# keeffEoghan/tendrils

Hardware: AMD Instinct MI355X
Metric: particle-steps/sec (16M particles per GPU) (higher is better)
Workload: dtype f32

## Files before the change

### include/tendrils_hip.h

```cpp
#ifndef TENDRILS_HIP_H
#define TENDRILS_HIP_H

#include <stddef.h>
#include <stdint.h>

#ifdef __cplusplus
extern "C" {
#endif

#define TH_ABI_VERSION 14

typedef int32_t th_status;
enum {
    TH_OK = 0,
    TH_ERR_INVALID = 1,
    TH_ERR_HIP = 2,
    TH_ERR_NO_DEVICE = 3,
    TH_ERR_UNSUPPORTED = 4
};

#define TH_INERT (-1000000.0f)

typedef struct th_context th_context;

// ... 224 lines not shown
    float alpha;
} th_blend_view;
th_status th_texture_upload(th_context *ctx, int32_t slot, int32_t format, const void *texels, int32_t w, int32_t h);
th_status th_texture_download(th_context *ctx, int32_t slot, void *texels);
th_status th_colormap_resize(th_context *ctx, int32_t w, int32_t h);
th_status th_colormap_shape(th_context *ctx, int32_t *w, int32_t *h);
th_status th_colormap_blend(th_context *ctx, const th_blend_view *views, int32_t n, int32_t gl_blend, int32_t clear);
th_status th_colormap_download(th_context *ctx, float *rgba);
th_status th_export_view_lines(th_context *ctx, const th_render_uniforms *u, float *lines, uint64_t capacity, uint64_t *count);
th_status th_draw_sharded(th_context *ctx, const th_deposit_uniforms *u, const th_render_uniforms *r, uint64_t *fragments);
th_status th_view_emit(th_context *ctx, const th_render_uniforms *u, uint64_t *count, void **keys_dev, void **colors_dev);
th_status th_view_merge(th_context *ctx, const void *keys_dev, const void *colors_dev, uint64_t count);
th_status th_view_device_ptr(th_context *ctx, void **dptr);
th_status th_draw_emit(th_context *ctx, const th_deposit_uniforms *u, const th_render_uniforms *r, uint64_t *count, void **keys_dev, void **colors_dev);
th_status th_draw_merge(th_context *ctx, const void *keys_dev, const void *colors_dev, uint64_t count);

typedef struct th_slot_order_info {
    int32_t sorted_buffers;
    int32_t steps_since_sort;
    uint64_t window_misses;
    uint64_t sorts;
} th_slot_order_info;
th_status th_slot_order(th_context *ctx, th_slot_order_info *out);

enum { TH_DRAW_AUTO = -1, TH_DRAW_STREAM = 0, TH_DRAW_BINS = 1 };
th_status th_draw_pipeline(th_context *ctx, int32_t which);
typedef struct th_draw_info {
    int32_t pipeline;
    int32_t reserved;
    uint64_t fragments, crowded_fragments;
    uint64_t sent_bytes, received_bytes;
} th_draw_info;
th_status th_draw_query(th_context *ctx, th_draw_info *out);

typedef struct th_flow_line_uniforms {
    float speed, rad, crestShape, speedLimit;
    float viewSize[2];
} th_flow_line_uniforms;

th_status th_flow_line_attributes(const float *points, const double *times, int32_t n, int32_t closed, int32_t capacity,
                                  int32_t *nverts, float *position, float *normal, float *miter, float *previous,
                                  float *time, float *dt);
th_status th_flow_lines(th_context *ctx, const th_flow_line_uniforms *u, const float *points, const double *times,
                        const int32_t *offsets, const int32_t *closed, int32_t nlines);

enum { TH_OPT_BUCKET = 0, TH_OPT_RESORT_STEPS = 1, TH_OPT_REBUCKET_STEPS = 2, TH_OPT_FUSE = 3, TH_OPT_GRAPH = 4,
       TH_OPT_FORCE_GENERIC = 5, TH_OPT_DRAW_REUSE = 6, TH_OPT_BINS_POOL = 7,
#ifdef TH_TESTING
       TH_OPT_INJECT_FAILURE = 8,
#endif
       TH_OPT_BINS_PAGES = 9, TH_OPT_ASYNC_SORT = 10, TH_OPT_SKIP_UNSEEN = 11, TH_OPT_SPAWN_CHUNK_ROWS = 12,
       TH_OPT_HASH_WINDOW = 13, TH_OPT_HASH_WINDOW_LAUNCHES = 14 };
th_status th_option_set(th_context *ctx, int32_t option, int64_t value);
th_status th_option_get(th_context *ctx, int32_t option, int64_t *value);

#ifdef __cplusplus
}
#endif
#endif
```

### tendrils_amd/_capi.py

```python
import ctypes as C
import os

HERE = os.path.dirname(os.path.abspath(__file__))
LIB_PATH = os.environ.get("TH_LIB") or os.path.join(HERE, "lib", "libtendrils_hip.so")

TH_OK = 0
TH_MODE_EXACT, TH_MODE_FAST = 0, 1
TH_STATE_F32, TH_STATE_F16 = 0, 1
TH_PASS_FLOW, TH_PASS_VIEW = 0, 1
TH_MAX_LINE_WIDTH = 64.0
TH_TARGET_RING, TH_TARGET_TARGETS, TH_SOURCE_FLOW, TH_SOURCE_IMAGE, TH_SOURCE_NONE = -1, -2, -3, -4, -5
TH_ERR_INVALID, TH_ERR_HIP, TH_ERR_NO_DEVICE, TH_ERR_UNSUPPORTED = 1, 2, 3, 4
INERT = -1000000.0


class TendrilsHipError(RuntimeError):

    def __init__(self, status, message):
        super().__init__("tendrils_hip status %d: %s" % (status, message))
        self.status = status


class Config(C.Structure):
    _fields_ = [("device", C.c_int32), ("width", C.c_int32), ("height", C.c_int32),
# ... 144 lines not shown
    "th_draw_sharded": (C.c_int32, [_ctx, C.POINTER(DepositUniforms), C.POINTER(RenderUniforms), C.POINTER(C.c_uint64)]),
    "th_view_device_ptr": (C.c_int32, [_ctx, C.POINTER(C.c_void_p)]),
    "th_state_gather": (C.c_int32, [_ctx, C.c_int32]),
    "th_state_gather_ptr": (C.c_int32, [_ctx, C.c_int32, C.POINTER(C.c_void_p)]),
    "th_spawn_sample_sharded": (C.c_int32, [_ctx, C.POINTER(SpawnSampleUniforms), C.c_int32, C.c_int32]),
    "th_spawn_query": (C.c_int32, [_ctx, C.POINTER(SpawnInfo)]),
    "th_stats": (C.c_int32, [_ctx, C.c_float, C.POINTER(Counters)]),
    "th_stats_async": (C.c_int32, [_ctx, C.c_float, C.POINTER(C.c_void_p)]),
    "th_comm_unique_id": (C.c_int32, [C.c_void_p]),
    "th_comm_loopback_id": (C.c_int32, [C.c_void_p]),
    "th_comm_init": (C.c_int32, [_ctx, C.c_void_p, C.c_int32, C.c_int32]),
    "th_comm_destroy": (C.c_int32, [_ctx]),
    "th_comm_query": (C.c_int32, [_ctx, C.POINTER(CommInfo)]),
    "th_stats_allreduce": (C.c_int32, [_ctx]),
    "th_stats_global": (C.c_int32, [_ctx, C.c_float, C.POINTER(Counters)]),
    "th_sync": (C.c_int32, [_ctx]),
    "th_stream": (C.c_int32, [_ctx, C.POINTER(C.c_void_p)]),
    "th_state_device_ptr": (C.c_int32, [_ctx, C.c_int32, C.POINTER(C.c_void_p)]),
    "th_timer_start": (C.c_int32, [_ctx]),
    "th_timer_stop": (C.c_int32, [_ctx, C.POINTER(C.c_float)]),
    "th_kernel_timing": (C.c_int32, [_ctx, C.c_int32]),
    "th_kernel_timing_read": (C.c_int32, [_ctx, C.POINTER(C.c_float), C.POINTER(C.c_int32)]),
    "th_slot_order": (C.c_int32, [_ctx, C.POINTER(SlotOrderInfo)]),
    "th_shapes": (C.c_int32, [_ctx, C.POINTER(ShapesInfo)]),
    "th_draw_pipeline": (C.c_int32, [_ctx, C.c_int32]),
    "th_draw_query": (C.c_int32, [_ctx, C.POINTER(DrawInfo)]),
    "th_option_set": (C.c_int32, [_ctx, C.c_int32, C.c_int64]),
    "th_option_get": (C.c_int32, [_ctx, C.c_int32, C.POINTER(C.c_int64)]),
    "th_line_width": (C.c_int32, [_ctx, C.c_int32, C.c_float]),
    "th_line_width_range": (C.c_int32, [_ctx, C.c_float, C.c_float]),
    "th_line_width_query": (C.c_int32, [_ctx, C.c_int32, C.POINTER(C.c_float), C.POINTER(C.c_float), C.POINTER(C.c_float)]),
    "th_view_draw": (C.c_int32, [_ctx, C.POINTER(RenderUniforms), C.POINTER(C.c_uint64)]),
    "th_draw": (C.c_int32, [_ctx, C.POINTER(DepositUniforms), C.POINTER(RenderUniforms), C.POINTER(C.c_uint64)]),
    "th_view_fill": (C.c_int32, [_ctx, _fp]),
    "th_view_clear": (C.c_int32, [_ctx]),
    "th_view_download": (C.c_int32, [_ctx, C.POINTER(C.c_uint8)]),
    "th_view_buffers": (C.c_int32, [_ctx, C.c_int32]),
    "th_view_bind": (C.c_int32, [_ctx, C.c_int32]),
    "th_view_copy": (C.c_int32, [_ctx, C.c_int32]),
    "th_view_step_buffers": (C.c_int32, [_ctx]),
    "th_colormap_upload": (C.c_int32, [_ctx, _fp, C.c_int32, C.c_int32]),
    "th_texture_upload": (C.c_int32, [_ctx, C.c_int32, C.c_int32, C.c_void_p, C.c_int32, C.c_int32]),
    "th_texture_download": (C.c_int32, [_ctx, C.c_int32, C.c_void_p]),
    "th_colormap_resize": (C.c_int32, [_ctx, C.c_int32, C.c_int32]),
    "th_colormap_shape": (C.c_int32, [_ctx, C.POINTER(C.c_int32), C.POINTER(C.c_int32)]),
    "th_colormap_blend": (C.c_int32, [_ctx, C.POINTER(BlendView), C.c_int32, C.c_int32, C.c_int32]),
# ... 82 lines not shown
```

### tendrils_amd/csrc/th_api.hip

```cpp
#include "th_ctx.hpp"

using namespace thi;

namespace {

thread_local std::string g_error;

void build_gradient_table(float4 *lut)
{
    for (int a = th::kLutMin; a <= th::kLutMax; ++a) {
        float p = th::permute_ref((float)a);
        float gx, gy, gz;
        th::gradient_ref(p, gx, gy, gz);
        lut[a - th::kLutMin] = make_float4(gx, gy, gz, 0.0f);
    }
}

void options_from_environment(th_options &o)
{
    auto number = [](const char *name, long long otherwise) { const char *e = getenv(name); return e && *e ? atoll(e) : otherwise; };
    o.bucket = (int)number("TH_BUCKET", -1);
    o.resort_steps = (int)number("TH_RESORT_STEPS", 64); if (o.resort_steps <= 0) o.resort_steps = 64;
    o.rebucket_steps = (int)number("TH_REBUCKET_STEPS", 256); if (o.rebucket_steps <= 0) o.rebucket_steps = 256;
    o.fuse = number("TH_FUSE", 1) != 0;
// ... 516 lines not shown
{
    TH_REQUIRE(c && out, "null argument");
    out->state_w = c->cfg.width; out->state_h = c->cfg.height;
    out->flow_w = c->fw; out->flow_h = c->fh;
    out->frames_w = c->frw; out->frames_h = c->frh;
    return TH_OK;
}

th_status th_option_set(th_context *c, int32_t option, int64_t value)
{
    if (th_status s = use(c)) return s;
    th_options &o = c->opt;
    switch (option) {
    case TH_OPT_BUCKET: TH_REQUIRE(value >= -1 && value <= 1, "TH_OPT_BUCKET takes -1, 0 or 1"); o.bucket = (int)value; break;
    case TH_OPT_RESORT_STEPS: TH_REQUIRE(value > 0 && value < (1 << 30), "TH_OPT_RESORT_STEPS must be positive"); o.resort_steps = (int)value; break;
    case TH_OPT_REBUCKET_STEPS: TH_REQUIRE(value > 0 && value < (1 << 30), "TH_OPT_REBUCKET_STEPS must be positive"); o.rebucket_steps = (int)value; break;
    case TH_OPT_FUSE: o.fuse = value != 0; break;
    case TH_OPT_GRAPH: o.graph = value != 0; break;
    case TH_OPT_FORCE_GENERIC: o.force_generic = value != 0; break;
    case TH_OPT_DRAW_REUSE: o.draw_reuse = value != 0; break;
    case TH_OPT_SKIP_UNSEEN: o.skip_unseen = value != 0; break;
    case TH_OPT_HASH_WINDOW: o.hash_window = value != 0; break;
    case TH_OPT_HASH_WINDOW_LAUNCHES: return fail(TH_ERR_INVALID, "TH_OPT_HASH_WINDOW_LAUNCHES is read-only");
    case TH_OPT_ASYNC_SORT: o.async_sort = value != 0; if (!o.async_sort) { if (th_status s = asort_drop(c)) return s; } break;
    case TH_OPT_BINS_POOL: TH_REQUIRE(value >= 0 && value < (1ll << 32), "TH_OPT_BINS_POOL out of range"); o.bins_pool = (uint32_t)value; break;
#ifdef TH_TESTING
    case TH_OPT_INJECT_FAILURE: TH_REQUIRE(value >= 0 && value <= 5, "TH_OPT_INJECT_FAILURE takes 0..5"); o.inject_failure = (int)value; break;
#endif
    case TH_OPT_SPAWN_CHUNK_ROWS: TH_REQUIRE(value >= 0 && value < (1 << 30), "TH_OPT_SPAWN_CHUNK_ROWS takes 0 (by the scratch budget) or a number of rows"); o.spawn_chunk_rows = (int)value; break;
    case TH_OPT_BINS_PAGES:
        TH_REQUIRE(value >= -(int64_t)th::kBinPagesLimit && value <= (int64_t)th::kBinPagesLimit && value != 1 && value != -1, "TH_OPT_BINS_PAGES takes 0, or 2..%u (negative: never widened)", th::kBinPagesLimit);
        o.bins_pages = (int)value;
        if (c->chunk_table) {
            TH_HIP(hipStreamSynchronize(c->stream));
            c->chunk_table.reset(); c->bin_mem.reset(); c->bin_capacity = 0; c->bin_max_pages = 0;
        }
        break;
    default: return fail(TH_ERR_INVALID, "unknown option %d", option);
    }
    clear_graphs(c);
    return TH_OK;
}

th_status th_option_get(th_context *c, int32_t option, int64_t *value)
{
    TH_REQUIRE(c && value, "null argument");
    const th_options &o = c->opt;
    switch (option) {
    case TH_OPT_BUCKET: *value = o.bucket; break;
    case TH_OPT_RESORT_STEPS: *value = o.resort_steps; break;
    case TH_OPT_REBUCKET_STEPS: *value = o.rebucket_steps; break;
    case TH_OPT_FUSE: *value = o.fuse; break;
    case TH_OPT_GRAPH: *value = o.graph; break;
    case TH_OPT_FORCE_GENERIC: *value = o.force_generic; break;
    case TH_OPT_DRAW_REUSE: *value = o.draw_reuse; break;
    case TH_OPT_ASYNC_SORT: *value = o.async_sort; break;
    case TH_OPT_SKIP_UNSEEN: *value = o.skip_unseen; break;
    case TH_OPT_HASH_WINDOW: *value = o.hash_window; break;
    case TH_OPT_HASH_WINDOW_LAUNCHES: *value = c->hash_window_launches; break;
    case TH_OPT_BINS_POOL: *value = o.bins_pool; break;
#ifdef TH_TESTING
    case TH_OPT_INJECT_FAILURE: *value = o.inject_failure; break;
#endif
    case TH_OPT_BINS_PAGES: *value = o.bins_pages; break;
    case TH_OPT_SPAWN_CHUNK_ROWS: *value = o.spawn_chunk_rows; break;
    default: return fail(TH_ERR_INVALID, "unknown option %d", option);
    }
    return TH_OK;
}

}
```

### tendrils_amd/csrc/th_ctx.hpp

```cpp
#pragma once
#include <hip/hip_runtime.h>

#include <algorithm>
#include <atomic>
#include <cmath>
#include <cstdarg>
#include <cstdio>
#include <cstdlib>
#include <cstring>
#include <limits>
#include <memory>
#include <mutex>
#include <new>
#include <string>
#include <vector>

#include "th_kernels.hpp"
#include "th_math.hpp"

namespace thi {
struct FlowLineScratch;
th_status fail(th_status code, const char *fmt, ...);
std::string &last_error();
}
// ... 67 lines not shown
    th::LogicParams key{};
    hipGraphExec_t exec = nullptr;
    DevBuf<float> times_dev;
    HostBuf<float> times_host;
    hipEvent_t copied = nullptr;
};

struct th_context {
    th_config cfg{};
    th_options opt{};
    hipStream_t stream = nullptr;
    std::vector<float4 *> ring;
    bool packed = false;
    DevBuf<float4> tmp[3];
    DevBuf<float4> flow;
    DevBuf<float2> flow_dec;
    DevBuf<float> flow3;
    int32_t fw = 0, fh = 0;
    DevBuf<float4> targets;
    bool targets_checked = true, targets_nonfinite = false;
    DevBuf<float4> lut_block;
    float4 *lut = nullptr;
    DevBuf<float4> win_block;
    long long hash_window_launches = 0;
    DevBuf<uchar4> frames[2];
    int32_t frw = 0, frh = 0;
    DevBuf<unsigned int> d_flag;
    DevBuf<th::StatsPartial> partials;
    DevBuf<th::StatsPartial> fused_parts;
    struct { bool valid = false; const float4 *buf = nullptr; float limit = 0.0f; uint32_t nparts = 0; } fused_stats;
    DevBuf<th_counters> d_counters;
    DevBuf<float4> x_halo;
    DevBuf<unsigned long long> x_counts;
    DevBuf<unsigned long long> x_keys;
    DevBuf<float4> x_colors;
    DevBuf<float4> gathered;
    const void *gathered_of = nullptr;
    DevBuf<char> sp_taps;
    DevBuf<uint32_t> sp_asked;
    DevBuf<float4> sp_answers;
    DevBuf<unsigned long long> sp_words;
    th_spawn_info last_spawn{};
    void *comm = nullptr;
    const th::Transport *transport = nullptr;
    DevBuf<uint32_t> d_status;
    DevBuf<uint32_t> own_mem;
// ... 284 lines not shown
```

### tendrils_amd/csrc/th_kernels.hip

```cpp
#include "th_kernels.hpp"
#include "th_math.hpp"
#include "th_logic.hpp"

#include <type_traits>
#include <cstdlib>

namespace th {


__global__ __launch_bounds__(256) void pack_state_kernel(uint2 *dst, const float4 *src, uint32_t n)
{
    for (uint32_t i = blockIdx.x * 256u + threadIdx.x; i < n; i += gridDim.x * 256u) dst[i] = pack_state(src[i]);
}

__global__ __launch_bounds__(256) void unpack_state_kernel(float4 *dst, const uint2 *src, uint32_t n)
{
    for (uint32_t i = blockIdx.x * 256u + threadIdx.x; i < n; i += gridDim.x * 256u) dst[i] = unpack_state(src[i]);
}

void launch_pack_state(void *dst, const float4 *src, uint32_t n, hipStream_t s)
{
    if (n) hipLaunchKernelGGL(pack_state_kernel, dim3(grid_for(n, 8)), dim3(256), 0, s, (uint2 *)dst, src, n);
}

// ... 164 lines not shown
        else fill_hash_tables(smem, p.lut);                                                                                   \
        __syncthreads();                                                                                                      \
    }                                                                                                                         \
    uint32_t idx, stride, end;                                                                                                \
    if constexpr (!BUCKETED) {                                                                                                \
        idx = blockIdx.x * 256u + threadIdx.x;                                                                                \
        stride = gridDim.x * 256u;                                                                                            \
        end = p.count;                                                                                                        \
    } else {                                                                                                                  \
        const uint32_t group = blockIdx.x & 7u, rank = blockIdx.x >> 3, per = (p.count + 7u) >> 3;                            \
        const uint32_t lo = group * per;                                                                                      \
        idx = lo + rank * 256u + threadIdx.x;                                                                                 \
        stride = (gridDim.x >> 3) * 256u;                                                                                     \
        end = lo + per < p.count ? lo + per : p.count;                                                                        \
    }                                                                                                                         \
    typename Fmt::Word nxt = Fmt::empty();                                                                                    \
    uint32_t npid = idx;                                                                                                      \
    [[maybe_unused]] bool first = true;                                                                                       \
    if (idx < end) {                                                                                                          \
        nxt = Fmt::load(p.in, idx);                                                                                           \
        if constexpr (BUCKETED) npid = __builtin_nontemporal_load(&p.perm[idx]);                                              \
    }                                                                                                                         \
    for (; idx < end; idx += stride) {                                                                                        \
        typename Fmt::Word w = nxt, wprev = w;                                                                                \
        const uint32_t pid = BUCKETED ? npid : idx;                                                                           \
        if (idx + stride < end) {                                                                                             \
            nxt = Fmt::load(p.in, idx + stride);                                                                              \
            if constexpr (BUCKETED) npid = __builtin_nontemporal_load(&p.perm[idx + stride]);                                 \
        }                                                                                                                     \
        float4 st = Fmt::decode(w);                                                                                           \
        for (uint32_t k = 0; k < p.nsteps; ++k) {                                                                             \
            if constexpr (!Fmt::packed) wprev = Fmt::encode(st);                                                              \
            else if (k + 1u == p.nsteps && k) wprev = Fmt::encode(st);                                                        \
            st = Fmt::quantize(integrate<FAST, NOISE, TARGET, POW2, false, true, !NOISE, WIN>(p, lut, st, pid, p.times[k], &tabs)); \
        }                                                                                                                     \
        if (!Fmt::packed || p.nsteps) w = Fmt::encode(st);                                                                    \
        Fmt::store(p.out_prev, idx, wprev);                                                                                   \
        Fmt::store(p.out, idx, w);                                                                                            \
        if constexpr (STATS) { stats_take(&p.stats_part[blockIdx.x * 4u + (threadIdx.x >> 6)], st, p.u.speedLimit, first); first = false; } \
    }                                                                                                                         \
    if constexpr (STATS) stats_none(&p.stats_part[blockIdx.x * 4u + (threadIdx.x >> 6)], first);

template <bool FAST, bool NOISE, bool TARGET, bool POW2, bool BUCKETED, bool STATS, bool WIN>
__global__ __launch_bounds__(256) void logic_fused_kernel(const LogicParams p) { TH_LOGIC_FUSED_LOOP(F32Texel) }

template <bool FAST, bool NOISE, bool TARGET, bool POW2, bool BUCKETED, bool STATS, bool WIN>
__global__ __launch_bounds__(256, 5) void logic_fused_packed_kernel(const LogicParams p) { TH_LOGIC_FUSED_LOOP(PackedTexel) }

int fused_grid(uint32_t count, bool bucketed)
{
    const uint32_t blocks = (count + 255u) / 256u;
    const uint32_t grid = bucketed ? 8u * ((((count + 7u) >> 3) + 255u) / 256u) : blocks;
    return (int)(grid ? grid : 1u);
}

void launch_logic_fused(const LogicParams &p, const LogicVariant &v, hipStream_t s)
{
    const bool packed = v.format == StateFormat::packed, bucketed = p.perm != nullptr;
    const int grid = fused_grid(p.count, bucketed);
    lift([&](auto fast, auto noise, auto target, auto pow2, auto bk, auto stats, auto window) {
        constexpr bool win = noise && !fast && window;
        hipLaunchKernelGGL((packed ? logic_fused_packed_kernel<fast, noise, target, pow2, bk, stats, win>
                                   : logic_fused_kernel<fast, noise, target, pow2, bk, stats, win>), dim3(grid), dim3(256), 0, s, p);
    }, v.mode == TH_MODE_FAST, v.noise, v.target, v.pow2, bucketed, p.stats_part != nullptr, p.win != nullptr);
}

TH_D uint32_t tile_key(const TileGeom &g, float px, float py, uint32_t pid)
{
    const uint32_t row = g.row0 + (g.pow2w ? pid >> g.log2w : pid / g.width);
    const uint32_t idle = ((g.row_draws[row >> 5] >> (row & 31u)) & 1u) ^ 1u;
    const bool taps = __builtin_fabsf(px) < __builtin_inff() && __builtin_fabsf(py) < __builtin_inff() &&
                      (px != kInert || py != kInert);
    if (!taps) return 2u * g.ntiles + idle;
    const int tx = (int)__builtin_amdgcn_fmed3f((px * g.view_x + 1.0f) * g.half_fw, 0.0f, g.fwm1);
    const int ty = (int)__builtin_amdgcn_fmed3f((py * g.view_y + 1.0f) * g.half_fh, 0.0f, g.fhm1);
    return 2u * ((uint32_t)(ty >> kTileShift) * g.tiles_x + (uint32_t)(tx >> kTileShift)) + idle;
}

struct WaveRuns { bool head; uint32_t rank, length, head_lane; };
TH_D WaveRuns wave_runs(uint32_t key, bool valid)
// ... 184 lines not shown
        Texel st[kRound];
        uint32_t pid[kRound];
#pragma unroll
        for (uint32_t q = 0; q < kRound; ++q) {
            const uint32_t s = base + (k0 + q) * 256u + threadIdx.x, at = s < b.count ? s : b.count - 1u;
            st[q] = __builtin_nontemporal_load(&reinterpret_cast<const Texel *>(b.state)[at]);
            pid[q] = __builtin_nontemporal_load(&ids[at]);
        }
#pragma unroll
        for (uint32_t q = 0; q < kRound; ++q) {
            const uint32_t s = base + (k0 + q) * 256u + threadIdx.x;
            const bool valid = s < b.count;
            float px, py;
            if constexpr (PACKED) { const float4 u = unpack_state(make_uint2(st[q].x, 0u)); px = u.x; py = u.y; }
            else { px = st[q].x; py = st[q].y; }
            const uint32_t key = valid ? tile_key(b.g, px, py, b.perm_in ? pid[q] : s) : 0u;
            const uint32_t d = tabled ? reserve_slots(bins, b.cursor, replica_of(blockIdx.x), key, valid)
                                      : reserve_slots(b.cursor, replica_of(blockIdx.x) + key, valid);
            if (valid) { reinterpret_cast<Texel *>(b.state_out)[d] = st[q]; b.perm_out[d] = b.perm_in ? pid[q] : s; }
        }
    }
}

template <typename Texel>
__global__ __launch_bounds__(256) void unpermute_state_kernel(Texel *dst, const Texel *src, const uint32_t *perm, uint32_t n)
{
    for (uint32_t s = blockIdx.x * 256u + threadIdx.x; s < n; s += gridDim.x * 256u) dst[perm[s]] = src[s];
}

template <typename Texel>
__global__ __launch_bounds__(256) void permute_state_kernel(Texel *dst, const Texel *src, const uint32_t *perm, uint32_t n)
{
    for (uint32_t s = blockIdx.x * 256u + threadIdx.x; s < n; s += gridDim.x * 256u) dst[s] = src[perm[s]];
}

static int tile_grid(uint32_t count) { return (int)((count + kTileChunk - 1) / kTileChunk); }

void launch_tile_hist(const TileSortParams &b, hipStream_t s)
{
    if (b.packed) hipLaunchKernelGGL(tile_hist_kernel<true>, dim3(tile_grid(b.count)), dim3(256), 0, s, b);
    else hipLaunchKernelGGL(tile_hist_kernel<false>, dim3(tile_grid(b.count)), dim3(256), 0, s, b);
}

void launch_tile_scan(const TileSortParams &b, hipStream_t s)
{
    const uint32_t bins = 2u * b.g.ntiles + 2u, grid = (bins + 255u) / 256u;
    hipLaunchKernelGGL(tile_scan_sum_kernel, dim3(grid), dim3(256), 0, s, b);
    hipLaunchKernelGGL(tile_scan_kernel, dim3(1), dim3(1024), 0, s, b);
    hipLaunchKernelGGL(tile_scan_place_kernel, dim3(grid), dim3(256), 0, s, b);
}

void launch_tile_scatter(const TileSortParams &b, hipStream_t s)
{
    if (b.packed) hipLaunchKernelGGL(tile_scatter_kernel<true>, dim3(tile_grid(b.count)), dim3(256), 0, s, b);
    else hipLaunchKernelGGL(tile_scatter_kernel<false>, dim3(tile_grid(b.count)), dim3(256), 0, s, b);
}

void launch_unpermute_state(float4 *dst, const float4 *src, const uint32_t *perm, uint32_t n, bool packed, hipStream_t s)
{
    if (packed) hipLaunchKernelGGL(unpermute_state_kernel<uint2>, dim3(grid_for(n, 8)), dim3(256), 0, s, reinterpret_cast<uint2 *>(dst),
                                   reinterpret_cast<const uint2 *>(src), perm, n);
    else hipLaunchKernelGGL(unpermute_state_kernel<float4>, dim3(grid_for(n, 8)), dim3(256), 0, s, dst, src, perm, n);
}

void launch_permute_state(float4 *dst, const float4 *src, const uint32_t *perm, uint32_t n, bool packed, hipStream_t s)
{
    if (packed) hipLaunchKernelGGL(permute_state_kernel<uint2>, dim3(grid_for(n, 8)), dim3(256), 0, s, reinterpret_cast<uint2 *>(dst),
                                   reinterpret_cast<const uint2 *>(src), perm, n);
    else hipLaunchKernelGGL(permute_state_kernel<float4>, dim3(grid_for(n, 8)), dim3(256), 0, s, dst, src, perm, n);
}

template <bool FAST, bool NOISE, bool TARGET, bool POW2, bool IN_TILED, bool SCATTER, bool COUNT>
__global__ __launch_bounds__(256, 5) void logic_sorted_kernel(const LogicParams p)
{
    __shared__ ChunkBins bins;
    __shared__ float4 smem[NOISE ? kHashVec + kLutSize : 1];
// ... 696 lines not shown
```

### tendrils_amd/csrc/th_kernels.hpp

```cpp
#pragma once
#include <string>

#include <hip/hip_runtime.h>
#include <stdint.h>

#include "../../include/tendrils_hip.h"

namespace th {

inline int grid_for(size_t n, int blocks_per_cu)
{
    size_t blocks = (n + 255) / 256;
    size_t cap = (size_t)256 * blocks_per_cu;
    return (int)(blocks < cap ? (blocks ? blocks : 1) : cap);
}

constexpr uint32_t kMaxFusedSteps = 32;
constexpr int kWinSpan = 286;
constexpr int kWinMaxCell = 8958;

constexpr uint32_t kTileChunk = 4096;
constexpr uint32_t kMaxTileBins = 8192;
constexpr uint32_t kSortReplicas = 64;
constexpr uint32_t kBinSlotsLog2 = 6, kBinSlots = 1u << kBinSlotsLog2;

struct TileGeom {
    float view_x, view_y, half_fw, half_fh, fwm1, fhm1;
    uint32_t tiles_x, ntiles;
    uint32_t width, log2w, pow2w, row0;
    const uint32_t *row_draws;
};

struct TileChunk { uint32_t start, count, tile, pad; };
struct ChunkRecord { uint32_t key[kBinSlots], count[kBinSlots]; };

struct LogicParams {
    const float4 *in;
    float4 *out;
    const float4 *flow;
    const float2 *flow_dec;
    const float *flow3;
    const float4 *targets;
    const float4 *lut;
    uint32_t count;
    uint32_t width;
    uint32_t log2w;
    uint32_t row0;
    float wf, hf;
    float inv_w, inv_h, inv_wh;
    int32_t fw, fh;
    float fwf, fhf, fwm1, fhm1, half_fw, half_fh;
    th_logic_uniforms u;
    float s2_cap;
    float pos_bound;
    const uint32_t *perm;
    TileGeom geom;
// ... 314 lines not shown
```

### tendrils_amd/csrc/th_logic.hpp

```cpp
#pragma once
#include "th_kernels.hpp"
#include "th_math.hpp"

namespace th {

typedef float v4f __attribute__((ext_vector_type(4)));
typedef unsigned v2u __attribute__((ext_vector_type(2)));
typedef float v2f __attribute__((ext_vector_type(2)));

TH_D uint32_t mad_u24_s(uint32_t a, uint32_t b, uint32_t c)
{
    uint32_t r;
    asm("v_mad_u32_u24 %0, %1, %2, %3" : "=v"(r) : "v"(a), "s"(b), "v"(c));
    return r;
}

TH_D float4 load_stream(const float4 *p)
{
    v4f v = __builtin_nontemporal_load(reinterpret_cast<const v4f *>(p));
    return make_float4(v.x, v.y, v.z, v.w);
}
TH_D void store_stream(float4 *p, float4 a)
{
    v4f v = {a.x, a.y, a.z, a.w};
// ... 213 lines not shown
    float d3 = mad<FAST>(g3.z, n.dz, mad<FAST>(g3.y, n.dy, g3.x * n.dx));
    float r = 42.0f * mad<FAST>(m3, d3, mad<FAST>(m2, d2, mad<FAST>(m1, d1, m0 * d0)));
    asm("" : "+v"(r) : "v"(g0.w), "v"(g1.w), "v"(g2.w), "v"(g3.w));
    return r;
}

constexpr int kTileShift = 5;
template <bool FAST, bool NOISE, bool TARGET, bool POW2, bool DECODED, bool PTAB = false, bool FLOW3 = false, bool WIN = false>
TH_D float4 integrate(const LogicParams &p, const float4 *lut, float4 st, uint32_t pid, float time,
                      const HashTables *tabs = nullptr)
{
    const th_logic_uniforms &u = p.u;
    float posx = st.x, posy = st.y, velx = st.z, vely = st.w;

    uint32_t x, y;
    if constexpr (POW2) { x = pid & (p.width - 1u); y = pid >> p.log2w; }
    else { y = pid / p.width; x = pid - y * p.width; }
    y += p.row0;

    static_assert(!WIN || (PTAB && !FAST), "the window: fused passes in exact mode");
    const float bound = WIN ? p.win_bound : p.pos_bound;
    bool in_domain = __builtin_fabsf(posx) < bound && __builtin_fabsf(posy) < bound;
    if (__builtin_expect(!in_domain, 0)) {
        if (!(posx != kInert || posy != kInert)) return st;
        if (!(__builtin_fabsf(posx) < __builtin_inff()) || !(__builtin_fabsf(posy) < __builtin_inff())) {
            const float q = __builtin_nanf("");
            return make_float4(q, q, q, q);
        }
        uint32_t rpid = pid;
        asm volatile("" : "+v"(rpid));
        uint32_t rx, ry;
        if constexpr (POW2) { rx = rpid & (p.width - 1u); ry = rpid >> p.log2w; }
        else { ry = rpid / p.width; rx = rpid - ry * p.width; }
        return logic_texel_ref(p, rx, ry + p.row0, st, rpid, time);
    }

    float fcx = (float)x + 0.5f, fcy = (float)y + 0.5f;
    float uvx, uvy, i;
    if constexpr (POW2) {
        uvx = fcx * p.inv_w; uvy = fcy * p.inv_h;
        i = (fcx + (fcy * p.wf)) * p.inv_wh;
    } else if constexpr (FAST) {
        uvx = fcx * p.inv_w; uvy = fcy * p.inv_h;
        i = mad<true>(fcy, p.wf, fcx) * p.inv_wh;
    } else {
        uvx = fcx / p.wf; uvy = fcy / p.hf;
        i = (fcx + (fcy * p.wf)) / (p.wf * p.hf);
    }

// ... 80 lines not shown
```

### tendrils_amd/csrc/th_order.hip

```cpp
#include "th_ctx.hpp"

using namespace thi;

namespace thi {

void destroy_graph(GraphEntry &g)
{
    if (g.exec) (void)hipGraphExecDestroy(g.exec);
    if (g.copied) (void)hipEventDestroy(g.copied);
    g = GraphEntry{};
}

void clear_graphs(th_context *c)
{
    if (!c->graphs.empty() && c->stream) (void)hipStreamSynchronize(c->stream);
    for (GraphEntry &g : c->graphs) destroy_graph(g);
    c->graphs.clear();
}

static uint32_t tile_count(const th_context *c, uint32_t *tiles_x)
{
    const uint32_t tx = ((uint32_t)c->fw + (1u << kTileShift) - 1u) >> kTileShift;
    const uint32_t ty = ((uint32_t)c->fh + (1u << kTileShift) - 1u) >> kTileShift;
    if (tiles_x) *tiles_x = tx;
// ... 163 lines not shown
    return TH_OK;
}

th_status asort_start(th_context *c, const th::TileGeom &g, float4 *src, int src_order)
{
    if (th_status s = sort_storage(c)) return s;
    if (!c->asort.dst) {
        TH_HIP(hipMalloc((void **)&c->asort.dst, c->texels() * sizeof(float4)));
        TH_HIP(hipEventCreateWithFlags(&c->asort.ready, hipEventDisableTiming));
        TH_HIP(hipEventCreateWithFlags(&c->asort.done, hipEventDisableTiming));
    }
    int order = -1;
    if (th_status s = free_order(c, &order)) return s;
    th_context::SlotOrder &o = c->orders[(size_t)order];
    th::TileSortParams b = sort_params(c, g, src, src_order >= 0 ? c->orders[(size_t)src_order].perm : nullptr, o);
    b.block_records = c->block_records;
    b.state_out = c->asort.dst;
    TH_HIP(hipEventRecord(c->asort.ready, c->stream));
    TH_HIP(hipStreamWaitEvent(c->side, c->asort.ready, 0));
    TH_HIP(hipMemsetAsync(b.hist, 0, kTileWords / 2 * sizeof(uint32_t), c->side));
    th::launch_tile_hist(b, c->side);
    th::launch_tile_scan(b, c->side);
    th::launch_tile_scatter(b, c->side);
    TH_HIP(hipGetLastError());
    TH_HIP(hipEventRecord(c->asort.done, c->side));
    ++c->sorts;
    o.stamp = c->sorts;
    c->counted.buf = nullptr;
    c->asort.pending = c->asort.valid = true;
    c->asort.src = src; c->asort.src_order = src_order; c->asort.order = order; c->asort.at_step = c->total_steps;
    return TH_OK;
}

th_status ensure_identity(th_context *c, bool *launched)
{
    if (launched) *launched = false;
    c->counted.buf = nullptr;
    if (!any_sorted(c)) return TH_OK;
    clear_graphs(c);
    for (float4 *&b : c->ring) {
        const int o = order_of(c, b);
        if (o < 0) continue;
        th::launch_unpermute_state(c->spare, b, c->orders[(size_t)o].perm, (uint32_t)c->texels(), c->packed, c->stream);
        ring_trade(c, b, c->spare, -1);
        if (launched) *launched = true;
    }
    TH_HIP(hipGetLastError());
    return TH_OK;
}

th_status begin_sort(th_context *c, const th::TileGeom &g, const float4 *state, const uint32_t *perm_in, int *order,
                     th::TileSortParams *params, bool have_hist)
{
    if (th_status s = sort_storage(c)) return s;
    if (th_status s = asort_drop(c)) return s;
    if (th_status s = free_order(c, order)) return s;
    th_context::SlotOrder &o = c->orders[(size_t)*order];
    th::TileSortParams b = sort_params(c, g, state, perm_in, o);
    b.block_records = have_hist ? nullptr : c->block_records;
    b.packed = c->packed ? 1u : 0u;
    if (!have_hist) {
        TH_HIP(hipMemsetAsync(b.hist, 0, kTileWords / 2 * sizeof(uint32_t), c->stream));
        th::launch_tile_hist(b, c->stream);
    }
    th::launch_tile_scan(b, c->stream);
    TH_HIP(hipMemsetAsync(c->tile_mem + kTileWords, 0, sizeof(uint32_t), c->stream));
    TH_HIP(hipGetLastError());
    c->steps_since_sort = 0;
    ++c->sorts;
    o.stamp = c->sorts;
    c->counted.buf = nullptr;
    if (params) *params = b;
    return TH_OK;
}

th_status fused_slots(th_context *c, bool may_sort, const th::TileGeom &g)
{
    if (!may_sort) return ensure_identity(c);
    const int o = order_of(c, c->ring[0]);
    if (o >= 0 && !order_stale(c, o, g) && c->steps_since_sort < c->opt.rebucket_steps) return TH_OK;
    float4 *cur = c->ring[0], *other = c->ring[1];
    set_order(c, other, -1);
    int fresh = -1;
    th::TileSortParams b;
    if (th_status s = begin_sort(c, g, cur, o >= 0 ? c->orders[(size_t)o].perm : nullptr, &fresh, &b)) return s;
    b.state_out = other;
// ... 27 lines not shown
}

}

extern "C" {

th_status th_slot_order(th_context *c, th_slot_order_info *out)
{
    if (th_status s = use(c)) return s;
    TH_REQUIRE(out, "null output");
    *out = th_slot_order_info{};
    out->sorted_buffers = (int32_t)c->buf_order.size();
    out->steps_since_sort = c->steps_since_sort;
    out->sorts = c->sorts;
    if (c->tile_mem) {
        uint32_t m = 0;
        TH_HIP(hipMemcpyAsync(&m, c->tile_mem + kTileWords, sizeof m, hipMemcpyDeviceToHost, c->stream));
        TH_HIP(hipStreamSynchronize(c->stream));
        out->window_misses = m;
    }
    return TH_OK;
}

}
```

### tendrils_amd/particles.py

```python
import ctypes as C

import numpy as np

from . import _capi
from ._capi import call


def defaults():
    return dict(shape=[64, 64], geomShape=None,
                logic=None, logicVert=None, logicFrag=None,
                render=None, renderVert=None, renderFrag=None)


class Program:

    COMPILE, SOURCE_KIND = "th_program_compile", "user"

    def __init__(self, kind, **fixed):
        self.kind = kind
        self.fixed = fixed
        self.uniforms = {}
        self.handle = None
        self.uniforms_struct = None

# ... 202 lines not shown
    def step_view_size(self, view_size):
        if view_size is None:
            call("th_step_program_view_size", self._ctx, None)
        else:
            call("th_step_program_view_size", self._ctx, (C.c_float * 2)(float(view_size[0]), float(view_size[1])))

    def draw(self, update=None, mode=None):
        return None

    def updateLogic(self, logicFrag):
        self.logic = logicFrag if isinstance(logicFrag, Program) else Program(LOGIC)

    def updateRender(self, *a):
        pass

    def sync(self):
        call("th_sync", self._ctx)

    def draw_pipeline(self, which):
        call("th_draw_pipeline", self._ctx, {"auto": -1, "stream": 0, "bins": 1}[which])

    OPTIONS = dict(bucket=0, resort_steps=1, rebucket_steps=2, fuse=3, graph=4, force_generic=5, draw_reuse=6, bins_pool=7,
                   inject_failure=8, bins_pages=9, async_sort=10, skip_unseen=11, spawn_chunk_rows=12,
                   hash_window=13, hash_window_launches=14)

    def option(self, name, value=None):
        if value is not None:
            call("th_option_set", self._ctx, self.OPTIONS[name], int(value))
        out = C.c_int64(0)
        call("th_option_get", self._ctx, self.OPTIONS[name], C.byref(out))
        return out.value

    def fetches_taps(self, source):
        if self.sharded_spawn != "auto":
            return bool(self.sharded_spawn)
        if source < 0 or self._global_height in (0, self.shape[1]):
            return False
        q = _capi.CommInfo()
        call("th_comm_query", self._ctx, C.byref(q))
        return bool(q.active)

    def deposit_flow(self, view_size, time, speed_limit):
        u = _capi.DepositUniforms(time=float(time), speedLimit=float(speed_limit))
        u.viewSize[0], u.viewSize[1] = float(view_size[0]), float(view_size[1])
        n = C.c_uint64(0)
        call("th_flow_deposit", self._ctx, C.byref(u), C.byref(n))
        return int(n.value)
# ... 122 lines not shown
```

Measured before the change: 217.0 billion.

## Add dense shared-memory tile sort path and restructure fused step loop

When the tile bin count fits in shared memory, histogram and scatter now use new dense kernels. These aggregate per-wave runs into LDS counters, then scatter slots and permutation using block-local ranks plus one global cursor atomic per bin, which should reduce global atomic traffic during re-sorting. The fused logic loop now writes the previous-state output inside the last iteration instead of re-encoding a saved word on every step, and it returns early when there are zero steps. It also adds asm barriers in the out-of-domain branch to steer codegen, plus a debug readback API and a counter for dense sorts.

```diff
diff --git a/include/tendrils_hip.h b/include/tendrils_hip.h
--- a/include/tendrils_hip.h
+++ b/include/tendrils_hip.h
@@ -270,6 +270,8 @@
     uint64_t sorts;
 } th_slot_order_info;
 th_status th_slot_order(th_context *ctx, th_slot_order_info *out);
+th_status th_slot_order_read(th_context *ctx, int32_t buffer, uint32_t *perm, uint32_t *chunks, uint32_t chunk_capacity,
+                             uint32_t *nchunks, void *slots, int32_t *sorted);
 
 enum { TH_DRAW_AUTO = -1, TH_DRAW_STREAM = 0, TH_DRAW_BINS = 1 };
 th_status th_draw_pipeline(th_context *ctx, int32_t which);
@@ -298,7 +300,7 @@
        TH_OPT_INJECT_FAILURE = 8,
 #endif
        TH_OPT_BINS_PAGES = 9, TH_OPT_ASYNC_SORT = 10, TH_OPT_SKIP_UNSEEN = 11, TH_OPT_SPAWN_CHUNK_ROWS = 12,
-       TH_OPT_HASH_WINDOW = 13, TH_OPT_HASH_WINDOW_LAUNCHES = 14 };
+       TH_OPT_HASH_WINDOW = 13, TH_OPT_HASH_WINDOW_LAUNCHES = 14, TH_OPT_DENSE_SORTS = 15 };
 th_status th_option_set(th_context *ctx, int32_t option, int64_t value);
 th_status th_option_get(th_context *ctx, int32_t option, int64_t *value);
 
diff --git a/tendrils_amd/_capi.py b/tendrils_amd/_capi.py
--- a/tendrils_amd/_capi.py
+++ b/tendrils_amd/_capi.py
@@ -190,6 +190,8 @@
     "th_kernel_timing": (C.c_int32, [_ctx, C.c_int32]),
     "th_kernel_timing_read": (C.c_int32, [_ctx, C.POINTER(C.c_float), C.POINTER(C.c_int32)]),
     "th_slot_order": (C.c_int32, [_ctx, C.POINTER(SlotOrderInfo)]),
+    "th_slot_order_read": (C.c_int32, [_ctx, C.c_int32, C.POINTER(C.c_uint32), C.POINTER(C.c_uint32), C.c_uint32, C.POINTER(C.c_uint32),
+                                       C.c_void_p, C.POINTER(C.c_int32)]),
     "th_shapes": (C.c_int32, [_ctx, C.POINTER(ShapesInfo)]),
     "th_draw_pipeline": (C.c_int32, [_ctx, C.c_int32]),
     "th_draw_query": (C.c_int32, [_ctx, C.POINTER(DrawInfo)]),
diff --git a/tendrils_amd/csrc/th_api.hip b/tendrils_amd/csrc/th_api.hip
--- a/tendrils_amd/csrc/th_api.hip
+++ b/tendrils_amd/csrc/th_api.hip
@@ -562,6 +562,7 @@
     case TH_OPT_SKIP_UNSEEN: o.skip_unseen = value != 0; break;
     case TH_OPT_HASH_WINDOW: o.hash_window = value != 0; break;
     case TH_OPT_HASH_WINDOW_LAUNCHES: return fail(TH_ERR_INVALID, "TH_OPT_HASH_WINDOW_LAUNCHES is read-only");
+    case TH_OPT_DENSE_SORTS: return fail(TH_ERR_INVALID, "TH_OPT_DENSE_SORTS is read-only");
     case TH_OPT_ASYNC_SORT: o.async_sort = value != 0; if (!o.async_sort) { if (th_status s = asort_drop(c)) return s; } break;
     case TH_OPT_BINS_POOL: TH_REQUIRE(value >= 0 && value < (1ll << 32), "TH_OPT_BINS_POOL out of range"); o.bins_pool = (uint32_t)value; break;
 #ifdef TH_TESTING
@@ -598,6 +599,7 @@
     case TH_OPT_SKIP_UNSEEN: *value = o.skip_unseen; break;
     case TH_OPT_HASH_WINDOW: *value = o.hash_window; break;
     case TH_OPT_HASH_WINDOW_LAUNCHES: *value = c->hash_window_launches; break;
+    case TH_OPT_DENSE_SORTS: *value = c->dense_sorts; break;
     case TH_OPT_BINS_POOL: *value = o.bins_pool; break;
 #ifdef TH_TESTING
     case TH_OPT_INJECT_FAILURE: *value = o.inject_failure; break;
diff --git a/tendrils_amd/csrc/th_ctx.hpp b/tendrils_amd/csrc/th_ctx.hpp
--- a/tendrils_amd/csrc/th_ctx.hpp
+++ b/tendrils_amd/csrc/th_ctx.hpp
@@ -113,6 +113,7 @@
     DevBuf<float4> lut_block;
     float4 *lut = nullptr;
     DevBuf<float4> win_block;
+    long long dense_sorts = 0;
     long long hash_window_launches = 0;
     DevBuf<uchar4> frames[2];
     int32_t frw = 0, frh = 0;
diff --git a/tendrils_amd/csrc/th_kernels.hip b/tendrils_amd/csrc/th_kernels.hip
--- a/tendrils_amd/csrc/th_kernels.hip
+++ b/tendrils_amd/csrc/th_kernels.hip
@@ -210,21 +210,24 @@
         if constexpr (BUCKETED) npid = __builtin_nontemporal_load(&p.perm[idx]);                                              \
     }                                                                                                                         \
     for (; idx < end; idx += stride) {                                                                                        \
-        typename Fmt::Word w = nxt, wprev = w;                                                                                \
+        const typename Fmt::Word w = nxt;                                                                                     \
         const uint32_t pid = BUCKETED ? npid : idx;                                                                           \
         if (idx + stride < end) {                                                                                             \
             nxt = Fmt::load(p.in, idx + stride);                                                                              \
             if constexpr (BUCKETED) npid = __builtin_nontemporal_load(&p.perm[idx + stride]);                                 \
         }                                                                                                                     \
         float4 st = Fmt::decode(w);                                                                                           \
-        for (uint32_t k = 0; k < p.nsteps; ++k) {                                                                             \
-            if constexpr (!Fmt::packed) wprev = Fmt::encode(st);                                                              \
-            else if (k + 1u == p.nsteps && k) wprev = Fmt::encode(st);                                                        \
-            st = Fmt::quantize(integrate<FAST, NOISE, TARGET, POW2, false, true, !NOISE, WIN>(p, lut, st, pid, p.times[k], &tabs)); \
-        }                                                                                                                     \
-        if (!Fmt::packed || p.nsteps) w = Fmt::encode(st);                                                                    \
-        Fmt::store(p.out_prev, idx, wprev);                                                                                   \
-        Fmt::store(p.out, idx, w);                                                                                            \
+        uint32_t left = p.nsteps;                                                                                             \
+        do {                                                                                                                  \
+            if (left == 1u) {                                                                                                 \
+                uint32_t at = idx;                                                                                            \
+                asm volatile("" : "+v"(at));                                                                                  \
+                if (Fmt::packed && p.nsteps == 1u) Fmt::store(p.out_prev, at, w);                                             \
+                else Fmt::store(p.out_prev, at, Fmt::encode(st));                                                             \
+            }                                                                                                                 \
+            st = Fmt::quantize(integrate<FAST, NOISE, TARGET, POW2, false, true, !NOISE, WIN>(p, lut, st, pid, p.times[p.nsteps - left], &tabs)); \
+        } while (--left);                                                                                                     \
+        Fmt::store(p.out, idx, Fmt::encode(st));                                                                              \
         if constexpr (STATS) { stats_take(&p.stats_part[blockIdx.x * 4u + (threadIdx.x >> 6)], st, p.u.speedLimit, first); first = false; } \
     }                                                                                                                         \
     if constexpr (STATS) stats_none(&p.stats_part[blockIdx.x * 4u + (threadIdx.x >> 6)], first);
@@ -244,6 +247,7 @@
 
 void launch_logic_fused(const LogicParams &p, const LogicVariant &v, hipStream_t s)
 {
+    if (!p.nsteps) return;
     const bool packed = v.format == StateFormat::packed, bucketed = p.perm != nullptr;
     const int grid = fused_grid(p.count, bucketed);
     lift([&](auto fast, auto noise, auto target, auto pow2, auto bk, auto stats, auto window) {
@@ -474,6 +478,91 @@
     }
 }
 
+constexpr uint32_t kDenseScatterSlots = 2048;
+static_assert(kDenseTileBins <= (1u << 20) && kDenseScatterSlots <= (1u << 12) && kTileChunk % kDenseScatterSlots == 0, "tile_scatter_dense_kernel: key << 12 | rank");
+
+template <bool PACKED>
+__global__ __launch_bounds__(256) void tile_hist_dense_kernel(const TileSortParams b)
+{
+    __shared__ uint32_t count[kDenseTileBins];
+    const uint32_t nbins = 2u * b.g.ntiles + 2u;
+    for (uint32_t k = threadIdx.x; k < nbins; k += 256u) count[k] = 0u;
+    const uint32_t base = blockIdx.x * kTileChunk;
+    float2 pos[kTileChunk / 256u];
+    uint32_t pid[kTileChunk / 256u];
+#pragma unroll
+    for (uint32_t k = 0; k < kTileChunk / 256u; ++k) {
+        const uint32_t s = base + k * 256u + threadIdx.x, at = s < b.count ? s : b.count - 1u;
+        pos[k] = slot_position<PACKED>(b.state, at);
+        pid[k] = b.perm_in ? b.perm_in[at] : at;
+    }
+    __syncthreads();
+#pragma unroll
+    for (uint32_t k = 0; k < kTileChunk / 256u; ++k) {
+        const uint32_t s = base + k * 256u + threadIdx.x;
+        const bool valid = s < b.count;
+        const uint32_t key = valid ? min(tile_key(b.g, pos[k].x, pos[k].y, pid[k]), nbins - 1u) : 0u;
+        const WaveRuns r = wave_runs(key, valid);
+        if (r.head) atomicAdd(&count[key], r.length);
+    }
+    __syncthreads();
+    const uint32_t rep = replica_of(blockIdx.x);
+    for (uint32_t k = threadIdx.x; k < nbins; k += 256u) {
+        const uint32_t n = count[k];
+        if (n) atomicAdd(&b.hist[rep + k], n);
+    }
+}
+
+template <bool PACKED>
+__global__ __launch_bounds__(256, 4) void tile_scatter_dense_kernel(const TileSortParams b)
+{
+    using Texel = std::conditional_t<PACKED, v2u, v4f>;
+    constexpr uint32_t kPer = kDenseScatterSlots / 256u;
+    __shared__ uint32_t table[kDenseTileBins];
+    const uint32_t nbins = 2u * b.g.ntiles + 2u;
+    for (uint32_t k = threadIdx.x; k < nbins; k += 256u) table[k] = 0u;
+    const uint32_t base = blockIdx.x * kDenseScatterSlots;
+    const uint32_t *ids = b.perm_in ? b.perm_in : reinterpret_cast<const uint32_t *>(b.state);
+    Texel st[kPer];
+    uint32_t pid[kPer], place[kPer];
+#pragma unroll
+    for (uint32_t q = 0; q < kPer; ++q) {
+        const uint32_t s = base + q * 256u + threadIdx.x, at = s < b.count ? s : b.count - 1u;
+        st[q] = __builtin_nontemporal_load(&reinterpret_cast<const Texel *>(b.state)[at]);
+        pid[q] = __builtin_nontemporal_load(&ids[at]);
+    }
+    __syncthreads();
+#pragma unroll
+    for (uint32_t q = 0; q < kPer; ++q) {
+        const uint32_t s = base + q * 256u + threadIdx.x;
+        const bool valid = s < b.count;
+        float px, py;
+        if constexpr (PACKED) { const float4 u = unpack_state(make_uint2(st[q].x, 0u)); px = u.x; py = u.y; }
+        else { px = st[q].x; py = st[q].y; }
+        const uint32_t key = valid ? min(tile_key(b.g, px, py, b.perm_in ? pid[q] : s), nbins - 1u) : 0u;
+        const WaveRuns r = wave_runs(key, valid);
+        uint32_t first = 0;
+        if (r.head) first = atomicAdd(&table[key], r.length);
+        place[q] = key << 12 | (__shfl(first, r.head_lane) + r.rank);
+    }
+    __syncthreads();
+    const uint32_t rep = replica_of(base / kTileChunk);
+    for (uint32_t k = threadIdx.x; k < nbins; k += 256u) {
+        const uint32_t n = table[k];
+        if (n) table[k] = atomicAdd(&b.cursor[rep + k], n);
+    }
+    __syncthreads();
+#pragma unroll
+    for (uint32_t q = 0; q < kPer; ++q) {
+        const uint32_t s = base + q * 256u + threadIdx.x;
+        if (s < b.count) {
+            const uint32_t d = table[place[q] >> 12] + (place[q] & 0xfffu);
+            reinterpret_cast<Texel *>(b.state_out)[d] = st[q];
+            b.perm_out[d] = b.perm_in ? pid[q] : s;
+        }
+    }
+}
+
 template <typename Texel>
 __global__ __launch_bounds__(256) void unpermute_state_kernel(Texel *dst, const Texel *src, const uint32_t *perm, uint32_t n)
 {
@@ -490,6 +579,11 @@
 
 void launch_tile_hist(const TileSortParams &b, hipStream_t s)
 {
+    if (tile_sort_dense(b.g)) {
+        if (b.packed) hipLaunchKernelGGL(tile_hist_dense_kernel<true>, dim3(tile_grid(b.count)), dim3(256), 0, s, b);
+        else hipLaunchKernelGGL(tile_hist_dense_kernel<false>, dim3(tile_grid(b.count)), dim3(256), 0, s, b);
+        return;
+    }
     if (b.packed) hipLaunchKernelGGL(tile_hist_kernel<true>, dim3(tile_grid(b.count)), dim3(256), 0, s, b);
     else hipLaunchKernelGGL(tile_hist_kernel<false>, dim3(tile_grid(b.count)), dim3(256), 0, s, b);
 }
@@ -504,6 +598,12 @@
 
 void launch_tile_scatter(const TileSortParams &b, hipStream_t s)
 {
+    if (tile_sort_dense(b.g)) {
+        const uint32_t grid = (b.count + kDenseScatterSlots - 1u) / kDenseScatterSlots;
+        if (b.packed) hipLaunchKernelGGL(tile_scatter_dense_kernel<true>, dim3(grid), dim3(256), 0, s, b);
+        else hipLaunchKernelGGL(tile_scatter_dense_kernel<false>, dim3(grid), dim3(256), 0, s, b);
+        return;
+    }
     if (b.packed) hipLaunchKernelGGL(tile_scatter_kernel<true>, dim3(tile_grid(b.count)), dim3(256), 0, s, b);
     else hipLaunchKernelGGL(tile_scatter_kernel<false>, dim3(tile_grid(b.count)), dim3(256), 0, s, b);
 }
diff --git a/tendrils_amd/csrc/th_kernels.hpp b/tendrils_amd/csrc/th_kernels.hpp
--- a/tendrils_amd/csrc/th_kernels.hpp
+++ b/tendrils_amd/csrc/th_kernels.hpp
@@ -21,6 +21,7 @@
 
 constexpr uint32_t kTileChunk = 4096;
 constexpr uint32_t kMaxTileBins = 8192;
+constexpr uint32_t kDenseTileBins = 4096;
 constexpr uint32_t kSortReplicas = 64;
 constexpr uint32_t kBinSlotsLog2 = 6, kBinSlots = 1u << kBinSlotsLog2;
 
@@ -32,6 +33,7 @@
 };
 
 struct TileChunk { uint32_t start, count, tile, pad; };
+inline bool tile_sort_dense(const TileGeom &g) { return 2u * g.ntiles + 2u <= kDenseTileBins; }
 struct ChunkRecord { uint32_t key[kBinSlots], count[kBinSlots]; };
 
 struct LogicParams {
diff --git a/tendrils_amd/csrc/th_logic.hpp b/tendrils_amd/csrc/th_logic.hpp
--- a/tendrils_amd/csrc/th_logic.hpp
+++ b/tendrils_amd/csrc/th_logic.hpp
@@ -259,9 +259,12 @@
     const float bound = WIN ? p.win_bound : p.pos_bound;
     bool in_domain = __builtin_fabsf(posx) < bound && __builtin_fabsf(posy) < bound;
     if (__builtin_expect(!in_domain, 0)) {
-        if (!(posx != kInert || posy != kInert)) return st;
+        float ix = posx, iy = posy;
+        asm volatile("" : "+v"(ix), "+v"(iy));
+        if (!(ix != kInert || iy != kInert)) return st;
         if (!(__builtin_fabsf(posx) < __builtin_inff()) || !(__builtin_fabsf(posy) < __builtin_inff())) {
-            const float q = __builtin_nanf("");
+            float q = __builtin_nanf("");
+            asm volatile("" : "+v"(q));
             return make_float4(q, q, q, q);
         }
         uint32_t rpid = pid;
diff --git a/tendrils_amd/csrc/th_order.hip b/tendrils_amd/csrc/th_order.hip
--- a/tendrils_amd/csrc/th_order.hip
+++ b/tendrils_amd/csrc/th_order.hip
@@ -209,6 +209,7 @@
     th::launch_tile_hist(b, c->side);
     th::launch_tile_scan(b, c->side);
     th::launch_tile_scatter(b, c->side);
+    if (th::tile_sort_dense(g)) ++c->dense_sorts;
     TH_HIP(hipGetLastError());
     TH_HIP(hipEventRecord(c->asort.done, c->side));
     ++c->sorts;
@@ -249,6 +250,7 @@
     if (!have_hist) {
         TH_HIP(hipMemsetAsync(b.hist, 0, kTileWords / 2 * sizeof(uint32_t), c->stream));
         th::launch_tile_hist(b, c->stream);
+        if (th::tile_sort_dense(g)) ++c->dense_sorts;
     }
     th::launch_tile_scan(b, c->stream);
     TH_HIP(hipMemsetAsync(c->tile_mem + kTileWords, 0, sizeof(uint32_t), c->stream));
@@ -322,4 +324,26 @@
     return TH_OK;
 }
 
-}
+th_status th_slot_order_read(th_context *c, int32_t buffer, uint32_t *perm, uint32_t *chunks, uint32_t chunk_capacity, uint32_t *nchunks,
+                             void *slots, int32_t *sorted)
+{
+    if (th_status s = use(c)) return s;
+    TH_REQUIRE(sorted && buffer >= 0 && (size_t)buffer < c->ring.size(), "th_slot_order_read: buffer out of range or null output");
+    TH_REQUIRE(!chunks || nchunks, "th_slot_order_read: chunks without nchunks");
+    const int o = order_of(c, c->ring[(size_t)buffer]);
+    *sorted = o >= 0 ? 1 : 0;
+    if (o < 0) return TH_OK;
+    const th_context::SlotOrder &so = c->orders[(size_t)o];
+    const size_t n = c->texels();
+    TH_HIP(hipStreamSynchronize(c->stream));
+    if (perm) TH_HIP(hipMemcpy(perm, so.perm, n * sizeof(uint32_t), hipMemcpyDeviceToHost));
+    if (nchunks) {
+        TH_HIP(hipMemcpy(nchunks, so.nchunks, sizeof(uint32_t), hipMemcpyDeviceToHost));
+        const size_t take = std::min<size_t>(std::min<size_t>(*nchunks, chunk_capacity), c->max_chunks);
+        if (chunks && take) TH_HIP(hipMemcpy(chunks, so.chunks, take * sizeof(th::TileChunk), hipMemcpyDeviceToHost));
+    }
+    if (slots) TH_HIP(hipMemcpy(slots, c->ring[(size_t)buffer], n * (c->packed ? sizeof(uint2) : sizeof(float4)), hipMemcpyDeviceToHost));
+    return TH_OK;
+}
+
+}
diff --git a/tendrils_amd/particles.py b/tendrils_amd/particles.py
--- a/tendrils_amd/particles.py
+++ b/tendrils_amd/particles.py
@@ -248,7 +248,7 @@
 
     OPTIONS = dict(bucket=0, resort_steps=1, rebucket_steps=2, fuse=3, graph=4, force_generic=5, draw_reuse=6, bins_pool=7,
                    inject_failure=8, bins_pages=9, async_sort=10, skip_unseen=11, spawn_chunk_rows=12,
-                   hash_window=13, hash_window_launches=14)
+                   hash_window=13, hash_window_launches=14, dense_sorts=15)
 
     def option(self, name, value=None):
         if value is not None:
```

Measured after the change: 220.8 billion (median of 6 runs). +1.8%, better.
